# NVlabs/EmerNeRF

Measured on NVIDIA H100. Metric: training rays/sec (8192-ray batch), higher is better.
Workload: dtype f32

## Files before the change

### emernerf_b200/csrc/grid.cu

```cuda
#include "common.cuh"
#include "grid_common.cuh"

namespace emer {

struct GridDescDev {
    emer_grid_desc g;
};

#ifndef EMER_GRID_DIAG_LEVEL_MAJOR
#define EMER_GRID_DIAG_LEVEL_MAJOR 0
#endif

template <int D>
__device__ __forceinline__ void load_point(const float* __restrict__ x, int64_t i, float (&p)[D]) {
    if constexpr (D == 4) {
        float4 v = __ldcs(reinterpret_cast<const float4*>(x) + i);
        p[0] = v.x; p[1] = v.y; p[2] = v.z; p[3] = v.w;
    } else {
#pragma unroll
        for (int d = 0; d < D; ++d) p[d] = __ldcs(x + i * D + d);
    }
}

template <int F>
struct Vec {
    float v[F];
};

template <int F>
__device__ __forceinline__ Vec<F> load_entry(const float* __restrict__ lt, uint32_t idx) {
    Vec<F> r;
    if constexpr (F == 4) {
        float4 t = __ldg(reinterpret_cast<const float4*>(lt) + idx);
        r.v[0] = t.x; r.v[1] = t.y; r.v[2] = t.z; r.v[3] = t.w;
    } else if constexpr (F == 2) {
        float2 t = __ldg(reinterpret_cast<const float2*>(lt) + idx);
        r.v[0] = t.x; r.v[1] = t.y;
    } else {
#pragma unroll
        for (int f = 0; f < F; ++f) r.v[f] = __ldg(lt + (size_t)idx * F + f);
    }
    return r;
}

template <int F>
__device__ __forceinline__ void red_add_entry(float* lt, uint32_t idx, const float (&v)[F]) {
    if constexpr (F == 4) {
        float* p = lt + (size_t)idx * 4;
        asm volatile("red.relaxed.gpu.global.add.v4.f32 [%0], {%1, %2, %3, %4};" ::"l"(p),
                     "f"(v[0]), "f"(v[1]), "f"(v[2]), "f"(v[3])
                     : "memory");
    } else if constexpr (F == 2) {
        float* p = lt + (size_t)idx * 2;
        asm volatile("red.relaxed.gpu.global.add.v2.f32 [%0], {%1, %2};" ::"l"(p), "f"(v[0]),
                     "f"(v[1])
                     : "memory");
    } else {
#pragma unroll
        for (int f = 0; f < F; ++f) atomicAdd(lt + (size_t)idx * F + f, v[f]);
    }
}

struct LevelGroups {
    uint64_t first, count;
    __device__ int first_of(int k) const { return (int)((first >> (4 * k)) & 15u); }
    __device__ int count_of(int k) const { return (int)((count >> (4 * k)) & 15u); }
};

template <int F>
constexpr int level_group() {
    return F == 4 ? 1 : 8 / F;
}

__device__ __forceinline__ int64_t out_vec(int64_t i, int l, int L, int64_t n) {
#if EMER_GRID_DIAG_LEVEL_MAJOR
    return (int64_t)l * n + i;
#else
    return i * L + l;
#endif
}

template <int D, int F, int G>
__global__ void __launch_bounds__(256) grid_fwd_kernel(const GridDescDev gd, const LevelGroups lg,
                                                       const float* __restrict__ x,
                                                       const float* __restrict__ table,
                                                       float* __restrict__ y, int64_t n) {
    const int64_t i = (int64_t)blockIdx.x * blockDim.x + threadIdx.x;
    const bool active = i < n;
    const emer_grid_desc& g = gd.g;
    const int L = g.n_levels;
    const int l0 = lg.first_of(blockIdx.y);
    const int cnt = lg.count_of(blockIdx.y);
    float p[D];
#pragma unroll
    for (int d = 0; d < D; ++d) p[d] = 0.0f;
    if (active) load_point<D>(x, i, p);
    const bool sector_pairs = !EMER_GRID_DIAG_LEVEL_MAJOR && F == 4 && cnt == 2 && !(L & 1);
    float4 held = make_float4(0.0f, 0.0f, 0.0f, 0.0f);
#pragma unroll
    for (int j = 0; j < (F == 4 ? 2 * G : G); ++j) {
        const int l = l0 + j;
        if (j >= cnt) break;
        const float scale = g.scale[l];
        const uint32_t res = g.resolution[l];
        const uint32_t off = g.offset[l];
        const uint32_t size = g.offset[l + 1] - off;
        const bool hashed = g.hashed[l] != 0;
        const float* lt = table + (size_t)off * F;
        uint32_t c0[D];
        float w[D];
        locate<D>(p, scale, c0, w);
        Vec<F> val[1 << D];
        float wt[1 << D];
#pragma unroll
        for (int c = 0; c < (1 << D); ++c) {
            uint32_t cc[D];
            corner_cell<D>(c, c0, cc);
            wt[c] = corner_weight<D>(c, w);
            val[c] = load_entry<F>(lt, grid_index<D>(cc, res, size, hashed));
        }
        float acc[F];
#pragma unroll
        for (int f = 0; f < F; ++f) acc[f] = 0.0f;
#pragma unroll
        for (int c = 0; c < (1 << D); ++c)
#pragma unroll
            for (int f = 0; f < F; ++f) acc[f] = fmaf(wt[c], val[c].v[f], acc[f]);
        if constexpr (F == 4) {
            const float4 v = make_float4(acc[0], acc[1], acc[2], acc[3]);
            if (!sector_pairs) {
                if (active) __stcs(reinterpret_cast<float4*>(y) + out_vec(i, l, L, n), v);
            } else if (j == 0) {
                held = v;
            } else {
                const bool odd = threadIdx.x & 1;
                const float4 send = odd ? held : v;
                float4 recv;
                recv.x = __shfl_xor_sync(0xffffffffu, send.x, 1);
                recv.y = __shfl_xor_sync(0xffffffffu, send.y, 1);
                recv.z = __shfl_xor_sync(0xffffffffu, send.z, 1);
                recv.w = __shfl_xor_sync(0xffffffffu, send.w, 1);
                const int64_t r0 = i & ~(int64_t)1;
                float4* yl = reinterpret_cast<float4*>(y) + l0 + (odd ? 1 : 0);
                if (r0 < n) __stcs(yl + r0 * L, odd ? recv : held);
                if (r0 + 1 < n) __stcs(yl + (r0 + 1) * L, odd ? v : recv);
            }
        } else if (active) {
            const int64_t q = out_vec(i, l, L, n);
            if constexpr (F == 2) {
                __stcs(reinterpret_cast<float2*>(y) + q, make_float2(acc[0], acc[1]));
            } else {
#pragma unroll
                for (int f = 0; f < F; ++f) __stcs(y + q * F + f, acc[f]);
            }
        }
    }
}

template <int D>
__global__ void grid_indices_kernel(const GridDescDev gd, const float* __restrict__ x,
                                    int32_t* __restrict__ out, int64_t n) {
    const int64_t i = (int64_t)blockIdx.x * blockDim.x + threadIdx.x;
    if (i >= n) return;
    const emer_grid_desc& g = gd.g;
    float p[D];
    load_point<D>(x, i, p);
    for (int l = 0; l < g.n_levels; ++l) {
        const uint32_t off = g.offset[l];
        const uint32_t size = g.offset[l + 1] - off;
        uint32_t c0[D];
        float w[D];
        locate<D>(p, g.scale[l], c0, w);
#pragma unroll
        for (int c = 0; c < (1 << D); ++c) {
            uint32_t cc[D];
            corner_cell<D>(c, c0, cc);
            out[(i * g.n_levels + l) * (1 << D) + c] =
                (int32_t)(off + grid_index<D>(cc, g.resolution[l], size, g.hashed[l] != 0));
        }
    }
}

template <int D, int F, int G>
__global__ void __launch_bounds__(256) grid_bwd_table_kernel(const GridDescDev gd, const LevelGroups lg,
                                                             const float* __restrict__ x,
                                                             const float* __restrict__ dy,
                                                             float* __restrict__ dtable, int64_t n) {
    const int64_t i = (int64_t)blockIdx.x * blockDim.x + threadIdx.x;
    const bool active = i < n;
    const int lane = threadIdx.x & 31;
    const emer_grid_desc& g = gd.g;
    const int L = g.n_levels;
    const int l0 = lg.first_of(blockIdx.y);
    const int cnt = lg.count_of(blockIdx.y);
    float p[D];
#pragma unroll
    for (int d = 0; d < D; ++d) p[d] = 0.0f;
    if (active) load_point<D>(x, i, p);
    const int64_t ia = active ? i : 0;
#pragma unroll
    for (int j = 0; j < (F == 4 ? 2 * G : G); ++j) {
        const int l = l0 + j;
        if (j >= cnt) break;
        float g_out[F];
#pragma unroll
        for (int f = 0; f < F; ++f) g_out[f] = 0.0f;
        const int64_t q = out_vec(ia, l, L, n);
        if (active) {
            if constexpr (F == 4) {
                const float4* dq = reinterpret_cast<const float4*>(dy) + q;
                float4 t = __ldcs(dq);
                g_out[0] = t.x; g_out[1] = t.y; g_out[2] = t.z; g_out[3] = t.w;
            } else if constexpr (F == 2) {
                float2 t = __ldcs(reinterpret_cast<const float2*>(dy) + q);
                g_out[0] = t.x; g_out[1] = t.y;
            } else {
#pragma unroll
                for (int f = 0; f < F; ++f) g_out[f] = __ldcs(dy + q * F + f);
            }
        }
        bool any = false;
#pragma unroll
        for (int f = 0; f < F; ++f) any |= (g_out[f] != 0.0f);
        const float scale = g.scale[l];
        const uint32_t res = g.resolution[l];
        const uint32_t off = g.offset[l];
        const uint32_t size = g.offset[l + 1] - off;
        const bool hashed = g.hashed[l] != 0;
        uint32_t c0[D];
        float w[D];
        locate<D>(p, scale, c0, w);
        uint32_t idx[1 << D];
#pragma unroll
        for (int c = 0; c < (1 << D); ++c) {
            uint32_t cc[D];
            corner_cell<D>(c, c0, cc);
            idx[c] = grid_index<D>(cc, res, size, hashed);
        }
        float* lt = dtable + (size_t)off * F;
        const uint64_t radix = (uint64_t)res + 1u;
        uint64_t span = 1;
#pragma unroll
        for (int d = 0; d < D; ++d) span *= radix;
        const bool keyable = span < 0xFFFFFFFFull;
        uint32_t key = 0xFFFFFFFFu;
        if (active && keyable) {
            key = 0;
#pragma unroll
            for (int d = D - 1; d >= 0; --d) key = key * (uint32_t)radix + c0[d];
        }
        const uint32_t prev = __shfl_up_sync(0xffffffffu, key, 1);
        const bool head = (lane == 0) || (key != prev) || !keyable;
        const unsigned heads = __ballot_sync(0xffffffffu, head);
        if (heads != 0xffffffffu) {
            const unsigned later = (lane == 31) ? 0u : (heads >> (lane + 1));
            const int run_end = later ? (lane + __ffs(later) - 1) : 31;
#pragma unroll
            for (int c = 0; c < (1 << D); ++c) {
                const float t = corner_weight<D>(c, w);
                float v[F];
#pragma unroll
                for (int f = 0; f < F; ++f) v[f] = t * g_out[f];
#pragma unroll
                for (int o = 1; o < 32; o <<= 1) {
#pragma unroll
                    for (int f = 0; f < F; ++f) {
                        const float u = __shfl_down_sync(0xffffffffu, v[f], o);
                        if (lane + o <= run_end) v[f] += u;
                    }
                }
                bool nz = false;
#pragma unroll
                for (int f = 0; f < F; ++f) nz |= (v[f] != 0.0f);
                if (head && active && nz) red_add_entry<F>(lt, idx[c], v);
            }
        } else if (any) {
#pragma unroll
            for (int c = 0; c < (1 << D); ++c) {
                const float t = corner_weight<D>(c, w);
                float v[F];
#pragma unroll
                for (int f = 0; f < F; ++f) v[f] = t * g_out[f];
                red_add_entry<F>(lt, idx[c], v);
            }
        }
    }
}

template <int D, int F>
__global__ void __launch_bounds__(256) grid_bwd_dx_kernel(const GridDescDev gd,
                                                          const float* __restrict__ x,
                                                          const float* __restrict__ table,
                                                          const float* __restrict__ dy,
                                                          float* __restrict__ dx, int64_t n) {
    const int64_t i = (int64_t)blockIdx.x * blockDim.x + threadIdx.x;
    if (i >= n) return;
    const emer_grid_desc& g = gd.g;
    const int L = g.n_levels;
    float p[D];
    load_point<D>(x, i, p);
    const float* dyo = dy + i * (int64_t)(L * F);
    float gx[D];
#pragma unroll
    for (int d = 0; d < D; ++d) gx[d] = 0.0f;
    for (int l = 0; l < L; ++l) {
        float g_out[F];
        if constexpr (F == 4) {
            float4 t = __ldg(reinterpret_cast<const float4*>(dyo) + l);
            g_out[0] = t.x; g_out[1] = t.y; g_out[2] = t.z; g_out[3] = t.w;
        } else if constexpr (F == 2) {
            float2 t = __ldg(reinterpret_cast<const float2*>(dyo) + l);
            g_out[0] = t.x; g_out[1] = t.y;
        } else {
#pragma unroll
            for (int f = 0; f < F; ++f) g_out[f] = __ldg(dyo + l * F + f);
        }
        bool any = false;
#pragma unroll
        for (int f = 0; f < F; ++f) any |= (g_out[f] != 0.0f);
        if (!any) continue;
        const float scale = g.scale[l];
        const uint32_t res = g.resolution[l];
        const uint32_t off = g.offset[l];
        const uint32_t size = g.offset[l + 1] - off;
        const bool hashed = g.hashed[l] != 0;
        const float* lt = table + (size_t)off * F;
        uint32_t c0[D];
        float w[D];
        locate<D>(p, scale, c0, w);
        float s[1 << D];
#pragma unroll
        for (int c = 0; c < (1 << D); ++c) {
            uint32_t cc[D];
            corner_cell<D>(c, c0, cc);
            Vec<F> v = load_entry<F>(lt, grid_index<D>(cc, res, size, hashed));
            float t = 0.0f;
#pragma unroll
            for (int f = 0; f < F; ++f) t = fmaf(g_out[f], v.v[f], t);
            s[c] = t;
        }
#pragma unroll
        for (int gdim = 0; gdim < D; ++gdim) {
            float acc = 0.0f;
#pragma unroll
            for (int c = 0; c < (1 << D); ++c) {
                if ((c >> gdim) & 1) continue;
                float t = scale;
#pragma unroll
                for (int d = 0; d < D; ++d) {
                    if (d == gdim) continue;
                    t = t * (((c >> d) & 1) ? w[d] : (1.0f - w[d]));
                }
                acc = fmaf(t, s[c | (1 << gdim)] - s[c], acc);
            }
            gx[gdim] += acc;
        }
    }
    if constexpr (D == 4) {
        reinterpret_cast<float4*>(dx)[i] = make_float4(gx[0], gx[1], gx[2], gx[3]);
    } else {
#pragma unroll
        for (int d = 0; d < D; ++d) dx[i * D + d] = gx[d];
    }
}

static int validate(const emer_grid_desc* g) {
    EMER_REQUIRE(g != nullptr, "grid desc is NULL");
    EMER_REQUIRE(g->n_dims == 3 || g->n_dims == 4, "grid: n_dims must be 3 or 4 (got %d)", g->n_dims);
    EMER_REQUIRE(g->n_levels >= 1 && g->n_levels <= EMER_MAX_LEVELS, "grid: n_levels %d out of range",
                 g->n_levels);
    EMER_REQUIRE(g->n_feat == 1 || g->n_feat == 2 || g->n_feat == 4, "grid: n_feat must be 1, 2 or 4 (got %d)",
                 g->n_feat);
    for (int l = 0; l < g->n_levels; ++l) {
        uint32_t size = g->offset[l + 1] - g->offset[l];
        EMER_REQUIRE(size > 0, "grid: empty level %d", l);
        EMER_REQUIRE(!g->hashed[l] || (size & (size - 1)) == 0, "grid: hashed level %d size %u not a power of two",
                     l, size);
    }
    return 0;
}

#define DISPATCH_DF(D_, F_, ...)                                   \
    if (g->n_dims == D_ && g->n_feat == F_) {                      \
        constexpr int D = D_;                                      \
        constexpr int F = F_;                                      \
        __VA_ARGS__;                                               \
    }

}

using namespace emer;

template <int F>
static int level_groups(const emer_grid_desc& g, bool forward, LevelGroups& lg) {
    constexpr uint64_t kScatterPairBytes = 24ull << 20;
    const int L = g.n_levels;
    int n = 0;
    for (int l = 0; l < L; ++n) {
        int c = level_group<F>();
        if (F == 4) {
            const bool pair = !(l & 1) && l + 1 < L &&
                              (forward ? !(L & 1)
                                       : (uint64_t)(g.offset[l + 2] - g.offset[l]) * F * 4 <= kScatterPairBytes);
            c = pair ? 2 : 1;
        }
        c = c < L - l ? c : L - l;
        lg.first |= (uint64_t)l << (4 * n);
        lg.count |= (uint64_t)c << (4 * n);
        l += c;
    }
    return n;
}

template <int D, int F>
static void launch_fwd(const GridDescDev& gd, const float* x, const float* table, float* y, int64_t n,
                       cudaStream_t st) {
    LevelGroups lg{0, 0};
    const int groups = level_groups<F>(gd.g, true, lg);
    const dim3 blocks((unsigned)ceil_div(n, 256), (unsigned)groups);
    grid_fwd_kernel<D, F, level_group<F>()><<<blocks, 256, 0, st>>>(gd, lg, x, table, y, n);
}

extern "C" int emer_grid_fwd(const emer_grid_desc* g, const float* x, const float* table, float* y,
                             int64_t n, void* stream) {
    if (int e = validate(g)) return e;
    if (n == 0) return 0;
    EMER_REQUIRE(x && table && y, "emer_grid_fwd: NULL pointer");
    EMER_REQUIRE(((uintptr_t)table & 15) == 0 && ((uintptr_t)y & 15) == 0 && ((uintptr_t)x & 15) == 0,
                 "emer_grid_fwd: pointers must be 16-byte aligned");
    GridDescDev gd{*g};
    cudaStream_t st = (cudaStream_t)stream;
    DISPATCH_DF(3, 1, (launch_fwd<D, F>(gd, x, table, y, n, st)))
    DISPATCH_DF(3, 2, (launch_fwd<D, F>(gd, x, table, y, n, st)))
    DISPATCH_DF(3, 4, (launch_fwd<D, F>(gd, x, table, y, n, st)))
    DISPATCH_DF(4, 1, (launch_fwd<D, F>(gd, x, table, y, n, st)))
    DISPATCH_DF(4, 2, (launch_fwd<D, F>(gd, x, table, y, n, st)))
    DISPATCH_DF(4, 4, (launch_fwd<D, F>(gd, x, table, y, n, st)))
    return check_launch("emer_grid_fwd");
}

extern "C" int emer_grid_indices(const emer_grid_desc* g, const float* x, int32_t* idx, int64_t n,
                                 void* stream) {
    if (int e = validate(g)) return e;
    if (n == 0) return 0;
    GridDescDev gd{*g};
    cudaStream_t st = (cudaStream_t)stream;
    const unsigned blocks = (unsigned)ceil_div(n, 256);
    if (g->n_dims == 3) grid_indices_kernel<3><<<blocks, 256, 0, st>>>(gd, x, idx, n);
    else grid_indices_kernel<4><<<blocks, 256, 0, st>>>(gd, x, idx, n);
    return check_launch("emer_grid_indices");
}

template <int D, int F>
static void launch_bwd(const GridDescDev& gd, const float* x, const float* table, const float* dy,
                       float* dtable, float* dx, int64_t n, cudaStream_t st) {
    const unsigned blocks = (unsigned)ceil_div(n, 256);
    if (dtable) {
        LevelGroups lg{0, 0};
        const dim3 grid(blocks, (unsigned)level_groups<F>(gd.g, false, lg));
        grid_bwd_table_kernel<D, F, level_group<F>()><<<grid, 256, 0, st>>>(gd, lg, x, dy, dtable, n);
    }
    if (dx) grid_bwd_dx_kernel<D, F><<<blocks, 256, 0, st>>>(gd, x, table, dy, dx, n);
}

extern "C" int emer_grid_bwd(const emer_grid_desc* g, const float* x, const float* table,
                             const float* dy, float* dtable, float* dx, int64_t n, void* stream) {
    if (int e = validate(g)) return e;
    if (n == 0 || (!dtable && !dx)) return 0;
    EMER_REQUIRE(x && dy, "emer_grid_bwd: NULL pointer");
    EMER_REQUIRE(!dx || table, "emer_grid_bwd: input gradient needs the table");
    EMER_REQUIRE(((uintptr_t)dy & 15) == 0 && ((uintptr_t)x & 15) == 0 && ((uintptr_t)dtable & 15) == 0 &&
                     ((uintptr_t)table & 15) == 0 && ((uintptr_t)dx & 15) == 0,
                 "emer_grid_bwd: pointers must be 16-byte aligned");
    GridDescDev gd{*g};
    cudaStream_t st = (cudaStream_t)stream;
    DISPATCH_DF(3, 1, (launch_bwd<D, F>(gd, x, table, dy, dtable, dx, n, st)))
    DISPATCH_DF(3, 2, (launch_bwd<D, F>(gd, x, table, dy, dtable, dx, n, st)))
    DISPATCH_DF(3, 4, (launch_bwd<D, F>(gd, x, table, dy, dtable, dx, n, st)))
    DISPATCH_DF(4, 1, (launch_bwd<D, F>(gd, x, table, dy, dtable, dx, n, st)))
    DISPATCH_DF(4, 2, (launch_bwd<D, F>(gd, x, table, dy, dtable, dx, n, st)))
    DISPATCH_DF(4, 4, (launch_bwd<D, F>(gd, x, table, dy, dtable, dx, n, st)))
    return check_launch("emer_grid_bwd");
}
```

### emernerf_b200/csrc/grid_common.cuh

```cuda
#pragma once
#include "common.cuh"

namespace emer {

template <int D>
__device__ __forceinline__ uint32_t grid_index(const uint32_t (&c)[D], uint32_t res, uint32_t size,
                                               bool hashed) {
    uint32_t idx = 0;
    if (hashed) {
        constexpr uint32_t P[4] = {1u, 2654435761u, 805459861u, 3674653429u};
#pragma unroll
        for (int d = 0; d < D; ++d) idx ^= c[d] * P[d];
        idx &= (size - 1u);
    } else {
        uint32_t stride = 1;
#pragma unroll
        for (int d = 0; d < D; ++d) {
            if (stride <= size) {
                idx += c[d] * stride;
                stride *= res;
            }
        }
        if (idx >= size) idx %= size;
    }
    return idx;
}

template <int D>
__device__ __forceinline__ void locate(const float (&p)[D], float scale, uint32_t (&c0)[D],
                                       float (&w)[D]) {
#pragma unroll
    for (int d = 0; d < D; ++d) {
        float pos = fmaf(scale, p[d], 0.5f);
        float fl = floorf(pos);
        c0[d] = (uint32_t)(int)fl;
        w[d] = pos - fl;
    }
}

template <int D>
__device__ __forceinline__ void corner_cell(int c, const uint32_t (&c0)[D], uint32_t (&cc)[D]) {
#pragma unroll
    for (int d = 0; d < D; ++d) cc[d] = c0[d] + ((c >> d) & 1);
}

template <int D>
__device__ __forceinline__ float corner_weight(int c, const float (&w)[D]) {
    float t = 1.0f;
#pragma unroll
    for (int d = 0; d < D; ++d) t = t * (((c >> d) & 1) ? w[d] : (1.0f - w[d]));
    return t;
}

}
```

### emernerf_b200/csrc/prop_level.cu

```cuda
#include "common.cuh"
#include "contract.cuh"
#include "grid_common.cuh"
#include "sampling.cuh"

namespace emer {

struct PropParams {
    emer_grid_desc g;
    const float* prev_s;
    const float* prev_cdf;
    const float* bias;
    const float* origins;
    const float* dirs;
    const float* aabb;
    const float* table;
    const float* w0;
    const float* b0;
    const float* w1;
    const float* b1;
    float* out_s;
    float* out_t;
    float* out_cdf;
    float* out_sigma;
    int64_t n_rays;
    int m1, n, stot_kind, unbounded;
    float s_min, s_max;
};

constexpr int PL_WARPS = 8;
constexpr int PL_MAX_EDGES = 257;
constexpr int PL_HID = 64;
constexpr int PL_MAX_IN = 16;

struct PlRay {
    float ox, oy, oz, dx, dy, dz, lo3[3], hi3[3];
};

__device__ __forceinline__ PlRay pl_load_ray(const float* origins, const float* dirs, const float* aabb, int64_t ray) {
    PlRay rc;
    rc.ox = __ldg(origins + ray * 3); rc.oy = __ldg(origins + ray * 3 + 1); rc.oz = __ldg(origins + ray * 3 + 2);
    rc.dx = __ldg(dirs + ray * 3); rc.dy = __ldg(dirs + ray * 3 + 1); rc.dz = __ldg(dirs + ray * 3 + 2);
    load_box(aabb, rc.lo3, rc.hi3);
    return rc;
}

template <int LF_T>
__device__ __forceinline__ void pl_encode(const emer_grid_desc& g, const float* __restrict__ table, int unbounded,
                                          const PlRay& rc, float t0, float t1, float (&xc)[3],
                                          float (&enc)[LF_T > 0 ? LF_T : PL_MAX_IN]) {
    const int L = LF_T > 0 ? LF_T : g.n_levels, F = LF_T > 0 ? 1 : g.n_feat;
    const float tt = t0 + t1;
    float pos[3] = {rc.ox + rc.dx * tt / 2.0f, rc.oy + rc.dy * tt / 2.0f, rc.oz + rc.dz * tt / 2.0f};
    float xn[3], mag;
    int amax;
    bool sel;
    contract_point(pos, rc.lo3, rc.hi3, unbounded, 1, xc, xn, mag, amax, sel);
#pragma unroll
    for (int l = 0; l < L; ++l) {
        const uint32_t res = g.resolution[l], off = g.offset[l], size = g.offset[l + 1] - off;
        const bool hashed = g.hashed[l] != 0;
        uint32_t c0[3];
        float w[3];
        locate<3>(xc, g.scale[l], c0, w);
        float acc[4] = {0.f, 0.f, 0.f, 0.f};
#pragma unroll
        for (int cc = 0; cc < 8; ++cc) {
            const float wt = corner_weight<3>(cc, w);
            uint32_t ci[3];
            corner_cell<3>(cc, c0, ci);
            const float* e = table + ((size_t)off + grid_index<3>(ci, res, size, hashed)) * F;
            if (LF_T > 0) acc[0] = fmaf(wt, __ldg(e), acc[0]);
            else for (int f = 0; f < F; ++f) acc[f] = fmaf(wt, __ldg(e + f), acc[f]);
        }
        if (LF_T > 0) enc[l] = acc[0];
        else for (int f = 0; f < F; ++f) enc[l * F + f] = acc[f];
    }
}

template <int LF>
__device__ __forceinline__ void pl_load_row(const float* __restrict__ row16, float (&w)[LF]) {
#pragma unroll
    for (int i = 0; i < LF; i += 4) {
        const float4 v = *reinterpret_cast<const float4*>(row16 + i);
        w[i] = v.x; w[i + 1] = v.y; w[i + 2] = v.z; w[i + 3] = v.w;
    }
}

template <int LF_T>
__global__ void __launch_bounds__(PL_WARPS * 32) prop_level_kernel(const PropParams p) {
    __shared__ float t_edges[PL_WARPS][PL_MAX_EDGES + 3];
    __shared__ __align__(16) float w0s[PL_HID * PL_MAX_IN];
    __shared__ float b0s[PL_HID], w1s[PL_HID];
    const int tid = threadIdx.x, lane = tid & 31, wid = tid >> 5;
    const int LF = LF_T > 0 ? LF_T : p.g.n_levels * p.g.n_feat;
    for (int e = tid; e < PL_HID * LF; e += PL_WARPS * 32) w0s[e] = __ldg(p.w0 + e);
    for (int e = tid; e < PL_HID; e += PL_WARPS * 32) { b0s[e] = __ldg(p.b0 + e); w1s[e] = __ldg(p.w1 + e); }
    __syncthreads();
    const float b1 = __ldg(p.b1);
    const int64_t ray = (int64_t)blockIdx.x * PL_WARPS + wid;
    if (ray >= p.n_rays) return;
    const int n = p.n, m1 = p.m1;

    const float bb = p.bias ? __ldg(p.bias + ray) : 0.5f;
    for (int k = lane; k <= n; k += 32) {
        int bin;
        const float s = resample_edge(p.prev_cdf + ray * m1, p.prev_s + ray * m1, m1, n, k, bb, bin);
        const float t = s_to_t(s, p.s_min, p.s_max, p.stot_kind);
        p.out_s[ray * (n + 1) + k] = s;
        p.out_t[ray * (n + 1) + k] = t;
        t_edges[wid][k] = t;
    }
    __syncwarp();

    const PlRay rc = pl_load_ray(p.origins, p.dirs, p.aabb, ray);
    float carry = 0.0f;
    for (int k0 = 0; k0 < n; k0 += 32) {
        const int k = k0 + lane;
        const bool ok = k < n;
        float xdelta = 0.0f;
        if (ok) {
            const float t0 = t_edges[wid][k], t1 = t_edges[wid][k + 1];
            float xc[3];
            float enc[LF_T > 0 ? LF_T : PL_MAX_IN];
            pl_encode<LF_T>(p.g, p.table, p.unbounded, rc, t0, t1, xc, enc);
            float raw = b1;
#pragma unroll 4
            for (int j = 0; j < PL_HID; ++j) {
                float h = b0s[j];
#pragma unroll
                for (int i = 0; i < LF; ++i) h = fmaf(w0s[j * LF + i], enc[i], h);
                h = h > 0.0f ? h : 0.0f;
                raw = fmaf(w1s[j], h, raw);
            }
            const float sigma = density_fwd(raw);
            xdelta = sigma * (t1 - t0);
            if (p.out_sigma) p.out_sigma[ray * n + k] = sigma;
        }
        const float incl = warp_scan_incl(xdelta, lane);
        const float e_excl = carry + (incl - xdelta);
        if (ok) p.out_cdf[ray * (n + 1) + k] = 1.0f - expf(-e_excl);
        carry += __shfl_sync(0xffffffffu, incl, 31);
    }
    if (lane == 0) p.out_cdf[ray * (n + 1) + n] = 1.0f;
}

struct PropBwdParams {
    emer_grid_desc g;
    const float* t_edges;
    const float* sigma;
    const float* d_cdf;
    const float* origins;
    const float* dirs;
    const float* aabb;
    const float* table;
    const float* w0;
    const float* b0;
    const float* w1;
    float* xc;
    float* d_enc;
    float* d_w0;
    float* d_b0;
    float* d_w1;
    float* d_b1;
    int64_t n_rays;
    int n, unbounded;
};

template <int LF>
__global__ void __launch_bounds__(PL_WARPS * 32) prop_level_bwd_kernel(const PropBwdParams p) {
    __shared__ float t_edges[PL_WARPS][PL_MAX_EDGES + 3];
    __shared__ float d_raw_s[PL_WARPS][PL_MAX_EDGES + 3];
    __shared__ __align__(16) float w0s[PL_HID * LF];
    __shared__ float b0s[PL_HID], w1s[PL_HID];
    __shared__ float red[PL_HID * LF + 2 * PL_HID + 1];
    const int tid = threadIdx.x, lane = tid & 31, wid = tid >> 5;
    for (int e = tid; e < PL_HID * LF; e += PL_WARPS * 32) w0s[e] = __ldg(p.w0 + e);
    for (int e = tid; e < PL_HID; e += PL_WARPS * 32) { b0s[e] = __ldg(p.b0 + e); w1s[e] = __ldg(p.w1 + e); }
    for (int e = tid; e < PL_HID * LF + 2 * PL_HID + 1; e += PL_WARPS * 32) red[e] = 0.0f;
    __syncthreads();
    float w0r[2][LF], b0r[2], w1r[2], acc_w0[2][LF], acc_b0[2], acc_w1[2];
#pragma unroll
    for (int u = 0; u < 2; ++u) {
        const int j = lane + 32 * u;
#pragma unroll
        for (int i = 0; i < LF; ++i) { w0r[u][i] = w0s[j * LF + i]; acc_w0[u][i] = 0.0f; }
        b0r[u] = b0s[j]; w1r[u] = w1s[j]; acc_b0[u] = 0.0f; acc_w1[u] = 0.0f;
    }
    float acc_b1 = 0.0f;
    const int n = p.n;
    for (int64_t ray = (int64_t)blockIdx.x * PL_WARPS + wid; ray < p.n_rays; ray += (int64_t)gridDim.x * PL_WARPS) {
        __syncwarp();
        for (int k = lane; k <= n; k += 32) t_edges[wid][k] = __ldg(p.t_edges + ray * (n + 1) + k);
        __syncwarp();
        float carry = 0.0f;
        for (int k0 = 0; k0 < n; k0 += 32) {
            const int k = k0 + lane;
            const bool ok = k < n;
            float xdelta = 0.0f;
            if (ok) xdelta = __ldg(p.sigma + ray * n + k) * (t_edges[wid][k + 1] - t_edges[wid][k]);
            const float incl = warp_scan_incl(xdelta, lane);
            const float e_excl = carry + (incl - xdelta);
            if (ok) d_raw_s[wid][k] = __ldg(p.d_cdf + ray * (n + 1) + k) * expf(-e_excl);
            carry += __shfl_sync(0xffffffffu, incl, 31);
        }
        __syncwarp();
        float tail = 0.0f;
        for (int k0 = ((n - 1) / 32) * 32; k0 >= 0; k0 -= 32) {
            const int k = k0 + (31 - lane);
            const bool ok = k < n;
            const float v = ok ? d_raw_s[wid][k] : 0.0f;
            const float incl = warp_scan_incl(v, lane);
            const float g_excl = tail + (incl - v);
            if (ok) {
                const float sg = __ldg(p.sigma + ray * n + k);
                d_raw_s[wid][k] = g_excl * (t_edges[wid][k + 1] - t_edges[wid][k]) * fminf(sg, 3269017.372472111f);
            }
            tail += __shfl_sync(0xffffffffu, incl, 31);
        }
        __syncwarp();
        const PlRay rc = pl_load_ray(p.origins, p.dirs, p.aabb, ray);
        for (int k0 = 0; k0 < n; k0 += 32) {
            const int k = k0 + lane;
            const bool ok = k < n;
            float enc[LF], d_enc[LF], xc[3] = {0.f, 0.f, 0.f};
            float d_raw = 0.0f;
#pragma unroll
            for (int i = 0; i < LF; ++i) { enc[i] = 0.0f; d_enc[i] = 0.0f; }
            if (ok) {
                pl_encode<LF>(p.g, p.table, p.unbounded, rc, t_edges[wid][k], t_edges[wid][k + 1], xc, enc);
                d_raw = d_raw_s[wid][k];
#pragma unroll 4
                for (int j = 0; j < PL_HID; ++j) {
                    float h = b0s[j];
                    float wr[LF];
                    pl_load_row<LF>(w0s + j * LF, wr);
#pragma unroll
                    for (int i = 0; i < LF; ++i) h = fmaf(wr[i], enc[i], h);
                    const float dh = h > 0.0f ? d_raw * w1s[j] : 0.0f;
#pragma unroll
                    for (int i = 0; i < LF; ++i) d_enc[i] = fmaf(dh, wr[i], d_enc[i]);
                }
                const int64_t pt = ray * n + k;
                p.xc[pt * 3] = xc[0]; p.xc[pt * 3 + 1] = xc[1]; p.xc[pt * 3 + 2] = xc[2];
#pragma unroll
                for (int i = 0; i < LF; i += 4)
                    *reinterpret_cast<float4*>(p.d_enc + pt * LF + i) = make_float4(d_enc[i], d_enc[i + 1], d_enc[i + 2], d_enc[i + 3]);
                acc_b1 += d_raw;
            }
            for (int sidx = 0; sidx < 32; ++sidx) {
                const float dr = __shfl_sync(0xffffffffu, d_raw, sidx);
                if (dr == 0.0f) continue;
                float e[LF];
#pragma unroll
                for (int i = 0; i < LF; ++i) e[i] = __shfl_sync(0xffffffffu, enc[i], sidx);
#pragma unroll
                for (int u = 0; u < 2; ++u) {
                    float h = b0r[u];
#pragma unroll
                    for (int i = 0; i < LF; ++i) h = fmaf(w0r[u][i], e[i], h);
                    const bool on = h > 0.0f;
                    const float dh = on ? dr * w1r[u] : 0.0f;
#pragma unroll
                    for (int i = 0; i < LF; ++i) acc_w0[u][i] = fmaf(dh, e[i], acc_w0[u][i]);
                    acc_b0[u] += dh;
                    acc_w1[u] = fmaf(dr, on ? h : 0.0f, acc_w1[u]);
                }
            }
        }
    }
#pragma unroll
    for (int u = 0; u < 2; ++u) {
        const int j = lane + 32 * u;
#pragma unroll
        for (int i = 0; i < LF; ++i) atomicAdd(&red[j * LF + i], acc_w0[u][i]);
        atomicAdd(&red[PL_HID * LF + j], acc_b0[u]);
        atomicAdd(&red[PL_HID * LF + PL_HID + j], acc_w1[u]);
    }
#pragma unroll
    for (int o = 16; o > 0; o >>= 1) acc_b1 += __shfl_xor_sync(0xffffffffu, acc_b1, o);
    if (lane == 0) atomicAdd(&red[PL_HID * LF + 2 * PL_HID], acc_b1);
    __syncthreads();
    for (int e = tid; e < PL_HID * LF + 2 * PL_HID + 1; e += PL_WARPS * 32) {
        const float v = red[e];
        float* dst = e < PL_HID * LF ? p.d_w0 + e
                   : e < PL_HID * LF + PL_HID ? p.d_b0 + (e - PL_HID * LF)
                   : e < PL_HID * LF + 2 * PL_HID ? p.d_w1 + (e - PL_HID * LF - PL_HID)
                   : p.d_b1;
        if (v != 0.0f) atomicAdd(dst, v);
    }
}

}

using namespace emer;

extern "C" int emer_prop_level(const emer_grid_desc* g, const float* prev_s, const float* prev_cdf, int m1, int n,
                               const float* bias, float s_min, float s_max, int stot_kind, const float* origins,
                               const float* dirs, const float* aabb6, int unbounded, const float* table,
                               const float* w0, const float* b0, const float* w1, const float* b1, float* out_s,
                               float* out_t, float* out_cdf, float* out_sigma, int64_t n_rays, void* stream) {
    if (n_rays == 0) return 0;
    EMER_REQUIRE(g && prev_s && prev_cdf && origins && dirs && aabb6 && table && w0 && b0 && w1 && b1 && out_s &&
                     out_t && out_cdf,
                 "emer_prop_level: NULL pointer");
    EMER_REQUIRE(g->n_dims == 3, "emer_prop_level: proposal grids are 3-D");
    EMER_REQUIRE(g->n_levels * g->n_feat <= PL_MAX_IN && g->n_feat <= 4, "emer_prop_level: at most %d grid features",
                 PL_MAX_IN);
    EMER_REQUIRE(m1 >= 2 && n >= 1 && n + 1 <= PL_MAX_EDGES, "emer_prop_level: n=%d out of range", n);
    PropParams p;
    p.g = *g;
    p.prev_s = prev_s; p.prev_cdf = prev_cdf; p.bias = bias; p.origins = origins; p.dirs = dirs; p.aabb = aabb6;
    p.table = table; p.w0 = w0; p.b0 = b0; p.w1 = w1; p.b1 = b1; p.out_s = out_s; p.out_t = out_t; p.out_cdf = out_cdf;
    p.out_sigma = out_sigma;
    p.n_rays = n_rays; p.m1 = m1; p.n = n; p.stot_kind = stot_kind; p.unbounded = unbounded; p.s_min = s_min; p.s_max = s_max;
    const unsigned blocks = (unsigned)ceil_div(n_rays, PL_WARPS);
    cudaStream_t st = (cudaStream_t)stream;
    const int lf = g->n_levels * g->n_feat;
    if (g->n_feat == 1 && lf == 8) prop_level_kernel<8><<<blocks, PL_WARPS * 32, 0, st>>>(p);
    else if (g->n_feat == 1 && lf == 4) prop_level_kernel<4><<<blocks, PL_WARPS * 32, 0, st>>>(p);
    else prop_level_kernel<0><<<blocks, PL_WARPS * 32, 0, st>>>(p);
    return check_launch("emer_prop_level");
}

extern "C" int emer_prop_level_bwd(const emer_grid_desc* g, const float* t_edges, const float* sigma, const float* d_cdf,
                                   int n, const float* origins, const float* dirs, const float* aabb6, int unbounded,
                                   const float* table, const float* w0, const float* b0, const float* w1, float* xc,
                                   float* d_enc, float* d_w0, float* d_b0, float* d_w1, float* d_b1, int64_t n_rays,
                                   void* stream) {
    if (n_rays == 0) return 0;
    EMER_REQUIRE(g && t_edges && sigma && d_cdf && origins && dirs && aabb6 && table && w0 && b0 && w1 && xc && d_enc &&
                     d_w0 && d_b0 && d_w1 && d_b1,
                 "emer_prop_level_bwd: NULL pointer");
    const int lf = g->n_levels * g->n_feat;
    EMER_REQUIRE(g->n_dims == 3 && g->n_feat == 1 && (lf == 8 || lf == 4),
                 "emer_prop_level_bwd: 3-D grids of 4 or 8 levels x 1 feature (got %d levels x %d)", g->n_levels, g->n_feat);
    EMER_REQUIRE(n >= 1 && n + 1 <= PL_MAX_EDGES, "emer_prop_level_bwd: n=%d out of range", n);
    EMER_REQUIRE(((uintptr_t)d_enc & 15) == 0, "emer_prop_level_bwd: d_enc must be 16-byte aligned");
    PropBwdParams p;
    p.g = *g;
    p.t_edges = t_edges; p.sigma = sigma; p.d_cdf = d_cdf; p.origins = origins; p.dirs = dirs; p.aabb = aabb6;
    p.table = table; p.w0 = w0; p.b0 = b0; p.w1 = w1; p.xc = xc; p.d_enc = d_enc; p.d_w0 = d_w0; p.d_b0 = d_b0;
    p.d_w1 = d_w1; p.d_b1 = d_b1; p.n_rays = n_rays; p.n = n; p.unbounded = unbounded;
    int64_t blocks = ceil_div(n_rays, PL_WARPS);
    const int64_t resident = (int64_t)sm_count() * 3;
    if (blocks > resident) blocks = resident;
    cudaStream_t st = (cudaStream_t)stream;
    if (lf == 8) prop_level_bwd_kernel<8><<<(unsigned)blocks, PL_WARPS * 32, 0, st>>>(p);
    else prop_level_bwd_kernel<4><<<(unsigned)blocks, PL_WARPS * 32, 0, st>>>(p);
    return check_launch("emer_prop_level_bwd");
}
```

Before: 2.570 million.

## Share corner gathers and scatters between paired lanes via warp shuffles

Adjacent lanes exchange point coordinates so each lane loads the low corners for one point and the high corners for its partner, then swaps the values back with xor-1 shuffles. Gathers from neighbouring x-corners should land in more coalesced or shared sectors. The same pairing is applied to the backward table scatter and to the proposal-level encoding, where inactive lanes are now clamped so every lane takes part in the shuffles. The proposal kernel also gains a min-blocks-per-SM launch bound of 2. The cost is extra shuffles, duplicate locate work, and redundant encodes on out-of-range lanes.

```diff
diff --git a/emernerf_b200/csrc/grid.cu b/emernerf_b200/csrc/grid.cu
--- a/emernerf_b200/csrc/grid.cu
+++ b/emernerf_b200/csrc/grid.cu
@@ -95,6 +95,9 @@
 #pragma unroll
     for (int d = 0; d < D; ++d) p[d] = 0.0f;
     if (active) load_point<D>(x, i, p);
+    float pq[D];
+#pragma unroll
+    for (int d = 0; d < D; ++d) pq[d] = F == 4 ? __shfl_xor_sync(0xffffffffu, p[d], 1) : 0.0f;
     const bool sector_pairs = !EMER_GRID_DIAG_LEVEL_MAJOR && F == 4 && cnt == 2 && !(L & 1);
     float4 held = make_float4(0.0f, 0.0f, 0.0f, 0.0f);
 #pragma unroll
@@ -113,11 +116,24 @@
         Vec<F> val[1 << D];
         float wt[1 << D];
 #pragma unroll
-        for (int c = 0; c < (1 << D); ++c) {
-            uint32_t cc[D];
-            corner_cell<D>(c, c0, cc);
-            wt[c] = corner_weight<D>(c, w);
-            val[c] = load_entry<F>(lt, grid_index<D>(cc, res, size, hashed));
+        for (int c = 0; c < (1 << D); ++c) wt[c] = corner_weight<D>(c, w);
+        if constexpr (F == 4) {
+            uint32_t c0q[D];
+            float wq[D];
+            locate<D>(pq, scale, c0q, wq);
+            float4 v4[1 << D];
+            gather_corner_pairs<D>(reinterpret_cast<const float4*>(lt), c0, c0q, res, size, hashed, v4);
+#pragma unroll
+            for (int c = 0; c < (1 << D); ++c) {
+                val[c].v[0] = v4[c].x; val[c].v[1] = v4[c].y; val[c].v[2] = v4[c].z; val[c].v[3] = v4[c].w;
+            }
+        } else {
+#pragma unroll
+            for (int c = 0; c < (1 << D); ++c) {
+                uint32_t cc[D];
+                corner_cell<D>(c, c0, cc);
+                val[c] = load_entry<F>(lt, grid_index<D>(cc, res, size, hashed));
+            }
         }
         float acc[F];
 #pragma unroll
@@ -197,6 +213,9 @@
 #pragma unroll
     for (int d = 0; d < D; ++d) p[d] = 0.0f;
     if (active) load_point<D>(x, i, p);
+    float pq[D];
+#pragma unroll
+    for (int d = 0; d < D; ++d) pq[d] = F == 4 ? __shfl_xor_sync(0xffffffffu, p[d], 1) : 0.0f;
     const int64_t ia = active ? i : 0;
 #pragma unroll
     for (int j = 0; j < (F == 4 ? 2 * G : G); ++j) {
@@ -273,6 +292,36 @@
 #pragma unroll
                 for (int f = 0; f < F; ++f) nz |= (v[f] != 0.0f);
                 if (head && active && nz) red_add_entry<F>(lt, idx[c], v);
+            }
+        } else if (F == 4 && !EMER_GRID_DIAG_XHIGH_REUSE) {
+            const bool odd = threadIdx.x & 1;
+            const bool any_q = __shfl_xor_sync(0xffffffffu, any, 1);
+            const bool any_r = odd ? any_q : any, any_s = odd ? any : any_q;
+            uint32_t c0q[D];
+            float wq[D];
+            locate<D>(pq, scale, c0q, wq);
+            uint32_t cr[D], cs[D];
+#pragma unroll
+            for (int d = 0; d < D; ++d) {
+                cr[d] = odd ? c0q[d] : c0[d];
+                cs[d] = odd ? c0[d] : c0q[d];
+            }
+#pragma unroll
+            for (int h = 0; h < (1 << (D - 1)); ++h) {
+                const float tl = corner_weight<D>(2 * h, w), th = corner_weight<D>(2 * h + 1, w);
+                float va[F], vb[F];
+#pragma unroll
+                for (int f = 0; f < F; ++f) {
+                    const float lo = tl * g_out[f], hi = th * g_out[f];
+                    const float r = __shfl_xor_sync(0xffffffffu, odd ? lo : hi, 1);
+                    va[f] = odd ? r : lo;
+                    vb[f] = odd ? hi : r;
+                }
+                uint32_t cc[D];
+                corner_cell<D>(2 * h + odd, cr, cc);
+                if (any_r) red_add_entry<F>(lt, grid_index<D>(cc, res, size, hashed), va);
+                corner_cell<D>(2 * h + odd, cs, cc);
+                if (any_s) red_add_entry<F>(lt, grid_index<D>(cc, res, size, hashed), vb);
             }
         } else if (any) {
 #pragma unroll
diff --git a/emernerf_b200/csrc/grid_common.cuh b/emernerf_b200/csrc/grid_common.cuh
--- a/emernerf_b200/csrc/grid_common.cuh
+++ b/emernerf_b200/csrc/grid_common.cuh
@@ -52,4 +52,57 @@
     return t;
 }
 
+#ifndef EMER_GRID_DIAG_XHIGH_REUSE
+#define EMER_GRID_DIAG_XHIGH_REUSE 0
+#endif
+
+__device__ __forceinline__ float shfl_xor1(float v) { return __shfl_xor_sync(0xffffffffu, v, 1); }
+__device__ __forceinline__ float4 shfl_xor1(float4 v) {
+    return make_float4(shfl_xor1(v.x), shfl_xor1(v.y), shfl_xor1(v.z), shfl_xor1(v.w));
 }
+
+template <int D, typename T>
+__device__ __forceinline__ void gather_corner_pairs(const T* __restrict__ lt, const uint32_t (&c0)[D],
+                                                    const uint32_t (&c0q)[D], uint32_t res, uint32_t size,
+                                                    bool hashed, T (&val)[1 << D]) {
+    constexpr int H = 1 << (D - 1);
+#if EMER_GRID_DIAG_XHIGH_REUSE
+    (void)c0q;
+#pragma unroll
+    for (int h = 0; h < H; ++h) {
+        uint32_t cc[D];
+        corner_cell<D>(2 * h, c0, cc);
+        val[2 * h] = __ldg(lt + grid_index<D>(cc, res, size, hashed));
+        val[2 * h + 1] = val[2 * h];
+    }
+#else
+    const bool odd = threadIdx.x & 1;
+    uint32_t cr[D], cs[D];
+#pragma unroll
+    for (int d = 0; d < D; ++d) {
+        cr[d] = odd ? c0q[d] : c0[d];
+        cs[d] = odd ? c0[d] : c0q[d];
+    }
+    T a[H], b[H];
+#pragma unroll
+    for (int h = 0; h < H; ++h) {
+        uint32_t cc[D];
+        corner_cell<D>(2 * h + odd, cr, cc);
+        a[h] = __ldg(lt + grid_index<D>(cc, res, size, hashed));
+    }
+#pragma unroll
+    for (int h = 0; h < H; ++h) {
+        uint32_t cc[D];
+        corner_cell<D>(2 * h + odd, cs, cc);
+        b[h] = __ldg(lt + grid_index<D>(cc, res, size, hashed));
+    }
+#pragma unroll
+    for (int h = 0; h < H; ++h) {
+        const T r = shfl_xor1(odd ? a[h] : b[h]);
+        val[2 * h] = odd ? r : a[h];
+        val[2 * h + 1] = odd ? b[h] : r;
+    }
+#endif
+}
+
+}
diff --git a/emernerf_b200/csrc/prop_level.cu b/emernerf_b200/csrc/prop_level.cu
--- a/emernerf_b200/csrc/prop_level.cu
+++ b/emernerf_b200/csrc/prop_level.cu
@@ -55,6 +55,9 @@
     int amax;
     bool sel;
     contract_point(pos, rc.lo3, rc.hi3, unbounded, 1, xc, xn, mag, amax, sel);
+    float xq[3];
+#pragma unroll
+    for (int d = 0; d < 3; ++d) xq[d] = LF_T > 0 ? shfl_xor1(xc[d]) : 0.0f;
 #pragma unroll
     for (int l = 0; l < L; ++l) {
         const uint32_t res = g.resolution[l], off = g.offset[l], size = g.offset[l + 1] - off;
@@ -63,14 +66,23 @@
         float w[3];
         locate<3>(xc, g.scale[l], c0, w);
         float acc[4] = {0.f, 0.f, 0.f, 0.f};
-#pragma unroll
-        for (int cc = 0; cc < 8; ++cc) {
-            const float wt = corner_weight<3>(cc, w);
-            uint32_t ci[3];
-            corner_cell<3>(cc, c0, ci);
-            const float* e = table + ((size_t)off + grid_index<3>(ci, res, size, hashed)) * F;
-            if (LF_T > 0) acc[0] = fmaf(wt, __ldg(e), acc[0]);
-            else for (int f = 0; f < F; ++f) acc[f] = fmaf(wt, __ldg(e + f), acc[f]);
+        if constexpr (LF_T > 0) {
+            uint32_t c0q[3];
+            float wq[3];
+            locate<3>(xq, g.scale[l], c0q, wq);
+            float val[8];
+            gather_corner_pairs<3>(table + off, c0, c0q, res, size, hashed, val);
+#pragma unroll
+            for (int cc = 0; cc < 8; ++cc) acc[0] = fmaf(corner_weight<3>(cc, w), val[cc], acc[0]);
+        } else {
+#pragma unroll
+            for (int cc = 0; cc < 8; ++cc) {
+                const float wt = corner_weight<3>(cc, w);
+                uint32_t ci[3];
+                corner_cell<3>(cc, c0, ci);
+                const float* e = table + ((size_t)off + grid_index<3>(ci, res, size, hashed)) * F;
+                for (int f = 0; f < F; ++f) acc[f] = fmaf(wt, __ldg(e + f), acc[f]);
+            }
         }
         if (LF_T > 0) enc[l] = acc[0];
         else for (int f = 0; f < F; ++f) enc[l * F + f] = acc[f];
@@ -87,7 +99,7 @@
 }
 
 template <int LF_T>
-__global__ void __launch_bounds__(PL_WARPS * 32) prop_level_kernel(const PropParams p) {
+__global__ void __launch_bounds__(PL_WARPS * 32, 2) prop_level_kernel(const PropParams p) {
     __shared__ float t_edges[PL_WARPS][PL_MAX_EDGES + 3];
     __shared__ __align__(16) float w0s[PL_HID * PL_MAX_IN];
     __shared__ float b0s[PL_HID], w1s[PL_HID];
@@ -118,11 +130,12 @@
         const int k = k0 + lane;
         const bool ok = k < n;
         float xdelta = 0.0f;
+        const int kc = ok ? k : n - 1;
+        const float t0 = t_edges[wid][kc], t1 = t_edges[wid][kc + 1];
+        float xc[3];
+        float enc[LF_T > 0 ? LF_T : PL_MAX_IN];
+        pl_encode<LF_T>(p.g, p.table, p.unbounded, rc, t0, t1, xc, enc);
         if (ok) {
-            const float t0 = t_edges[wid][k], t1 = t_edges[wid][k + 1];
-            float xc[3];
-            float enc[LF_T > 0 ? LF_T : PL_MAX_IN];
-            pl_encode<LF_T>(p.g, p.table, p.unbounded, rc, t0, t1, xc, enc);
             float raw = b1;
 #pragma unroll 4
             for (int j = 0; j < PL_HID; ++j) {
@@ -226,8 +239,12 @@
             float d_raw = 0.0f;
 #pragma unroll
             for (int i = 0; i < LF; ++i) { enc[i] = 0.0f; d_enc[i] = 0.0f; }
-            if (ok) {
-                pl_encode<LF>(p.g, p.table, p.unbounded, rc, t_edges[wid][k], t_edges[wid][k + 1], xc, enc);
+            const int kc = ok ? k : n - 1;
+            pl_encode<LF>(p.g, p.table, p.unbounded, rc, t_edges[wid][kc], t_edges[wid][kc + 1], xc, enc);
+            if (!ok) {
+#pragma unroll
+                for (int i = 0; i < LF; ++i) enc[i] = 0.0f;
+            } else {
                 d_raw = d_raw_s[wid][k];
 #pragma unroll 4
                 for (int j = 0; j < PL_HID; ++j) {
```

New measurement: 2.662 million (median of 6 runs). 1.04x the previous value.
